# Arsham-001/tsu-emulator

Hardware: AMD Instinct MI355X
Metric: spin-updates/sec on L×L 2D Ising Gibbs sweep; achieved HBM GB/s vs peak (higher is better)
Workload: dtype int8

## Files before the change

### tsu-emulator_amd/csrc/ising2d_tiled.hip

```cpp
#include "ising2d.h"

#include <type_traits>
#include <vector>

typedef short v2s __attribute__((ext_vector_type(2)));
typedef unsigned short v2us __attribute__((ext_vector_type(2)));

struct TiledParams {
    const int8_t* src;
    int8_t* dst;
    long long pitch;
    int rows, nchunks;
    int cols;
    int q_shift;
    int tile_h;
    int flex_ty;
    int r_begin, r_end;
    long long row0, total_rows;
    int wrap_rows, ghost;
    int k;
    int tiles_x;
    int ty_first, ty_stride;
    uint32_t k0, k1, sweep0, tag_hi, tag_lo;
    uint32_t tblH0, tblH1, tblL0, tblL1;
// ... 205 lines not shown
template <int NO>
static __device__ __forceinline__ void edge_rows(const Rows2Ctx& c, int to_wrap, int tr, int& rga, int& rgb) {
    constexpr int SPAN = 2 * ((NO - 1 + 63) / NO) + 1;
    const int s_off = to_wrap > 0 ? c.rg_tile0 : c.rg_tile0 - c.total_rows;
    rga = tr + s_off;
    rgb = rga + 1;
    if (__builtin_expect((uint32_t)(to_wrap - 1) < (uint32_t)SPAN, 0)) {
        rga = tr + c.rg_tile0;
        asm volatile("" : "+v"(rga));
        rgb = rga + 1;
        if (rga >= c.total_rows) rga -= c.total_rows;
        if (rgb >= c.total_rows) rgb -= c.total_rows;
    }
}

constexpr int TBL2_OCTETS = 13;
constexpr uint32_t TBL2_LDS_ADDR = 0;

template <typename E, int NO>
struct TilePlanes {
    E* base;
    __device__ __forceinline__ E& at(int pl, int r, int o) const { return base[(2 * r + pl) * NO + o]; }
};

template <int NO, int KAPPA, int P0, bool EDGE, bool OPEN, bool SEAM>
static __device__ __forceinline__ void pair_step(const Rows2Ctx& c, const PhiloxKeys& K, uint32_t hs, uint32_t y0, uint32_t a, int rg, int to_wrap,
                                                 uint32_t cq) {
    constexpr int RS = 2 * NO * 8;
    constexpr int DO = (KAPPA ? NO : -NO) * 8;
    const uint64_t R0 = lds_ld<uint64_t>(a), R1 = lds_ld<uint64_t>(a + RS);
    const uint64_t R2 = lds_ld<uint64_t>(a + 2 * RS), R3 = lds_ld<uint64_t>(a + 3 * RS);
    const uint32_t A0 = SEAM ? 0u : (P0 ? lds_ld<volatile uint32_t>(a + RS + 8) : lds_ld<uint32_t>(a + RS - 4));
    const uint32_t A1 = SEAM ? 0u : (P0 ? lds_ld<uint32_t>(a + 2 * RS - 4) : lds_ld<volatile uint32_t>(a + 2 * RS + 8));
    const uint64_t Na = SEAM ? lds_ld<uint64_t>(a + RS + (P0 ? 8 : -8)) : 0ull;
    const uint64_t Nb = SEAM ? lds_ld<uint64_t>(a + 2 * RS + (P0 ? -8 : 8)) : 0ull;
    __builtin_amdgcn_sched_barrier(0);
    int rga = rg, rgb = rg + 1;
    if (EDGE) edge_rows<NO>(c, to_wrap, rg, rga, rgb);
    constexpr bool EARLY = !OPEN;
    auto counts = [&]() -> PairCounts {
        const uint32_t C0l = (uint32_t)R1, C0h = (uint32_t)(R1 >> 32), C1l = (uint32_t)R2, C1h = (uint32_t)(R2 >> 32);
        uint32_t S0l = P0 ? __builtin_amdgcn_alignbyte(C0h, C0l, 1) : __builtin_amdgcn_alignbyte(C0l, A0, 3);
        uint32_t S0h = P0 ? __builtin_amdgcn_alignbyte(A0, C0h, 1) : __builtin_amdgcn_alignbyte(C0h, C0l, 3);
        uint32_t S1l = P0 ? __builtin_amdgcn_alignbyte(C1l, A1, 3) : __builtin_amdgcn_alignbyte(C1h, C1l, 1);
        uint32_t S1h = P0 ? __builtin_amdgcn_alignbyte(C1h, C1l, 3) : __builtin_amdgcn_alignbyte(A1, C1h, 1);
        if (SEAM) {
            const uint64_t nxa = (Na & 0xFFull) << c.sh_next, pva = (Na >> c.sh_prev) & 0xFFull;
            const uint64_t nxb = (Nb & 0xFFull) << c.sh_next, pvb = (Nb >> c.sh_prev) & 0xFFull;
            const uint64_t Sa = P0 ? ((R1 >> 8) | nxa) : ((R1 << 8) | pva);
            const uint64_t Sb = P0 ? ((R2 << 8) | pvb) : ((R2 >> 8) | nxb);
            S0l = (uint32_t)Sa; S0h = (uint32_t)(Sa >> 32);
            S1l = (uint32_t)Sb; S1h = (uint32_t)(Sb >> 32);
        }
        const uint32_t ml = C0l + C1l, mh = C0h + C1h;
        return PairCounts{(uint32_t)R0 + ml + S0l, (uint32_t)(R0 >> 32) + mh + S0h, (uint32_t)R3 + ml + S1l, (uint32_t)(R3 >> 32) + mh + S1h};
    };
    PairCounts n;
    PairThr T;
    const u32x4 w0 = philox_vk(cq, (uint32_t)rga, c.rmask, y0, hs, c.tag_hi, K);
    if constexpr (EARLY) {
        __builtin_amdgcn_sched_barrier(0);
        n = counts();
        T = pair_thresholds(n, c.tbl2);
        __builtin_amdgcn_sched_barrier(0);
    }
    const u32x4 w1 = philox_vk(cq, (uint32_t)rgb, c.rmask, y0, hs, c.tag_hi, K);
    __builtin_amdgcn_sched_barrier(0);
    if constexpr (!EARLY) n = counts();
    const uint32_t cnt0l = n.c0l, cnt0h = n.c0h, cnt1l = n.c1l, cnt1h = n.c1h;
    u32x4 d0, d1;
    uint32_t edge_a = 0, edge_b = 0;
    if (OPEN) {
        const bool ea = rga == 0 || rga == c.last_row, eb = rgb == 0 || rgb == c.last_row;
        const bool la = !P0 && c.lft, ra = c.rgt && c.r_par == (uint32_t)P0, lb = P0 && c.lft, rb = c.rgt && c.r_par != (uint32_t)P0;
        d0 = compare_octet_open(w0, cnt0l, cnt0h, c, ea, la, ra);
        d1 = compare_octet_open(w1, cnt1l, cnt1h, c, eb, lb, rb);
        edge_a = (ea ? 1u : 0u) | (la ? 2u : 0u) | (ra ? 4u : 0u) | (c.r_slot << 4);
        edge_b = (eb ? 1u : 0u) | (lb ? 2u : 0u) | (rb ? 4u : 0u) | (c.r_slot << 4);
    } else {
        d0 = compare_octet_thr(w0, T.t);
        d1 = compare_octet_thr(w1, T.t + 4);
// ... 4 lines not shown
        if (has_zero_field(d1)) d1 = resolve_ties(d1, w1, cnt1l, cnt1h, c.s_thr, cq, (uint32_t)rgb & c.rmask, hs, c.tag_lo, c.k0, c.k1, edge_b);
    }
    uint64_t n0 = pack_flags(d0), n1 = pack_flags(d1);
    if (OPEN) {
        n0 = (rga < 0 || rga > c.last_row) ? 0 : (n0 & (P0 ? c.vm_o : c.vm_e));
        n1 = (rgb < 0 || rgb > c.last_row) ? 0 : (n1 & (P0 ? c.vm_e : c.vm_o));
    }
    if (SEAM) {
        n0 &= c.vm_e;
        n1 &= c.vm_e;
    }
    lds_st<uint64_t>(a + RS + DO, n0);
    lds_st<uint64_t>(a + 2 * RS + DO, n1);
}

template <int NO, int RL, int KAPPA, int P0, bool EDGE, bool OPEN, bool SEAM = false>
static __device__ __forceinline__ void sweep_pairs(const Rows2Ctx& c, const PhiloxKeys& K, uint32_t hs, uint32_t y0, uint32_t a, int rg, int n, bool tail,
                                                   uint32_t cq) {
    int to_wrap = EDGE ? c.wrap_tr - __builtin_amdgcn_readfirstlane(rg) : 0;
    bool live = true;
#pragma unroll 1
    for (int i = n; i >= 0; --i) {
        if (i == 0) live = tail;
        asm volatile("" : "+v"(a), "+v"(rg));
        if (live) pair_step<NO, KAPPA, P0, EDGE, OPEN, SEAM>(c, K, hs, y0, a, rg, to_wrap, cq);
        a += 2 * RL * 2 * NO * 8;
        rg += 2 * RL;
        to_wrap -= 2 * RL;
    }
}


static __device__ __forceinline__ uint32_t nib_shift_next(uint32_t X, uint32_t N) {
    const uint32_t hi = (N << 4) | __builtin_amdgcn_ubfe(X, 4u, 4u);
    return __builtin_amdgcn_alignbit(hi, X, 8);
}
static __device__ __forceinline__ uint32_t nib_shift_prev(uint32_t X, uint32_t M) {
    const uint32_t w = ((X << 4) & 0x10000000u) | (M >> 4);
    return __builtin_amdgcn_alignbit(X, w, 24);
}
static __device__ __forceinline__ uint32_t nib_shift_next_seam(uint32_t X, uint32_t N, int pos) {
    return nib_shift_next(X, 0u) | ((N & 0xFu) << pos);
}
// ... 76 lines not shown
static __device__ __forceinline__ void sweep_pairs_nib(const Rows2Ctx& c, const PhiloxKeys& K, uint32_t hs, uint32_t y0, uint32_t a, int rg, int n, bool tail,
                                                       uint32_t cq) {
    int to_wrap = EDGE ? c.wrap_tr - __builtin_amdgcn_readfirstlane(rg) : 0;
    bool live = true;
#pragma unroll 1
    for (int i = n; i >= 0; --i) {
        if (i == 0) live = tail;
        asm volatile("" : "+v"(a), "+v"(rg));
        if (live) pair_step_nib<NO, KAPPA, P0, EDGE, OPEN, SEAM>(c, K, hs, y0, a, rg, to_wrap, cq);
        a += 2 * RL * 2 * NO * 4;
        rg += 2 * RL;
        to_wrap -= 2 * RL;
    }
}

template <int NO, int RL, int KAPPA, int P0, bool EDGE, bool OPEN, bool SEAM, bool NIB>
static __device__ __forceinline__ void half_sweep(const Rows2Ctx& c, const PhiloxKeys& K, int TR, uint32_t sweep, int s, uint32_t a_thr, int al,
                                                  uint32_t cq) {
    constexpr int ES = NIB ? 4 : 8;
    const int hsi = 2 * s + KAPPA;
    __syncthreads();
    if (al < RL) {
        const int npairs = (TR - 2 - 2 * hsi) / 2;
        const int n = __builtin_amdgcn_readfirstlane(npairs / RL);
        const bool tail = al < npairs - n * RL;
        const uint32_t a = a_thr + (uint32_t)(hsi * 2 * NO * ES + (KAPPA ? 0 : NO * ES));
        int rg;
        if (EDGE) {
            rg = 1 + hsi + 2 * al;
        } else {
            int rgf = c.rg_tile0 + 1 + hsi;
            if (!OPEN && rgf >= c.total_rows) rgf -= c.total_rows;
            rg = rgf + 2 * al;
        }
        const uint32_t hs = 2u * sweep + (uint32_t)KAPPA;
        const uint32_t y0 = philox_y0(hs, c.k0);
        if constexpr (NIB) sweep_pairs_nib<NO, RL, KAPPA, P0, EDGE, OPEN, SEAM>(c, K, hs, y0, a, rg, n, tail, cq);
        else sweep_pairs<NO, RL, KAPPA, P0, EDGE, OPEN, SEAM>(c, K, hs, y0, a, rg, n, tail, cq);
    }
}

template <int NO, int RL, int P0, bool EDGE, bool OPEN, bool SEAM, bool NIB>
static __device__ __forceinline__ void sweep_generation(const Rows2Ctx& c, const PhiloxKeys& K, int TR, uint32_t sweep_g, int kg, uint32_t a_thr,
                                                        int al, uint32_t cq) {
#pragma unroll 1
    for (int s = 0; s < kg; ++s) {
        half_sweep<NO, RL, 0, P0, EDGE, OPEN, SEAM, NIB>(c, K, TR, sweep_g + (uint32_t)s, s, a_thr, al, cq);
        half_sweep<NO, RL, 1, P0, EDGE, OPEN, SEAM, NIB>(c, K, TR, sweep_g + (uint32_t)s, s, a_thr, al, cq);
    }
}

static __device__ __forceinline__ void xst(uint64_t* p, uint64_t v) { __hip_atomic_store(p, v, __ATOMIC_RELAXED, __HIP_MEMORY_SCOPE_AGENT); }
static __device__ __forceinline__ uint64_t xld(const uint64_t* p) { return __hip_atomic_load(p, __ATOMIC_RELAXED, __HIP_MEMORY_SCOPE_AGENT); }

struct ResidentParams {
    uint64_t* xbuf;
    uint32_t gen0;
    int* err;
    int n_gen, k_last, tiles_y;
    int wrap_y;
    int wrap_x;
    long long* dbg;
};

template <int HT, int WO, int THREADS, bool OPEN = false, bool RESIDENT = false, bool NIB = false>
static __device__ __forceinline__ void tile_body(const TiledParams& p, const int8_t* __restrict__ src, int8_t* __restrict__ dst,
                                                 const int k, const uint32_t sweep0, const int tx, const int ty, uint64_t* lds,
                                                 const PhiloxKeys& K, const ResidentParams* R = nullptr) {
    constexpr int NO = WO + 2;
    constexpr int RLMAX = THREADS / NO;
    int H, row_off;
    tile_rows(p, ty, row_off, H);
    const int TR = H + 4 * k;
    constexpr int RL = RLMAX;
    using E = typename std::conditional<NIB, uint32_t, uint64_t>::type;
    uint64_t* const guard = lds + TBL2_OCTETS;
    const TilePlanes<E, NO> P{reinterpret_cast<E*>(guard + 1)};
// ... 97 lines not shown
    const bool ragged = !OPEN && v_last != 0;
    const int seam_site = v_last - 1;
    const int seam_pos = NIB ? 8 * (seam_site & 3) + 4 * (seam_site >> 2) : 8 * seam_site, last_pos = NIB ? 28 : 56;
    c.sh_next = (ragged && cqi == p.nchunks - 1) ? seam_pos : last_pos;
    c.sh_prev = (ragged && cqi == 0) ? seam_pos : last_pos;
    int w0 = (q0 - 1) % p.nchunks;
    if (w0 < 0) w0 += p.nchunks;
    const bool seam = ragged && (w0 == 0 || w0 + NO - 1 >= p.nchunks - 1);
    if constexpr (OPEN) {
        asm volatile("v_mov_b32 %0, %1" : "=v"(c.tblH0) : "s"(p.tblH0));
        asm volatile("v_mov_b32 %0, %1" : "=v"(c.tblH1) : "s"(p.tblH1));
        asm volatile("v_mov_b32 %0, %1" : "=v"(c.tblL0) : "s"(p.tblL0));
        asm volatile("v_mov_b32 %0, %1" : "=v"(c.tblL1) : "s"(p.tblL1));
    }

    const int n_gen = RESIDENT ? R->n_gen : 1;
    long long tl0 = 0, tl[4] = {0, 0, 0, 0};
    const bool timing = RESIDENT && R->dbg && tid == 0;
    if (timing) tl0 = wall_clock64();
#define RES_MARK(q)                         \
    if (timing) {                           \
        const long long now_ = wall_clock64(); \
        tl[q] += now_ - tl0;                \
        tl0 = now_;                         \
    }
    volatile int& s_fail = *reinterpret_cast<volatile int*>(guard);
    if (RESIDENT && tid == 0) s_fail = 0;

    const int n_tb = 2 * k * WO, n_lr = H;
    const int xstride = 2 * n_tb + 2 * p.tile_h;
    const int wi = (p.nchunks + p.q_shift - q0) < WO ? (p.nchunks + p.q_shift - q0) : WO;
    constexpr uint64_t TAG_MASK = NIB ? 0xFFFFFFFF00000000ull : 0xFEFEull, FLAG_MASK = NIB ? 0x11111111ull : 0x0101010101010101ull;
// ... 52 lines not shown
            ad[it] = oc == 0 ? X_dl + e + w_l - 1 : (oc == wi + 1 ? X_dr + e : X_d + e + oc - 1);
            const bool col_ok = o == 0 ? has_l : (o == wi + 1 ? has_r : o <= wi);
            nu[it] = i < 2 * k * NO && has_u && col_ok;
            nd[it] = i < 2 * k * NO && has_d && col_ok;
            vu[it] = xld(au[it]);
            vd[it] = xld(ad[it]);
        }
#pragma unroll
        for (int it = 0; it < SI; ++it) {
            const int i = tid + it * THREADS, ic = i < n_lr ? i : 0;
            nl[it] = i < n_lr && has_l;
            nr[it] = i < n_lr && has_r;
            vl[it] = xld(X_l + 2 * n_tb + n_lr + ic);
            vr[it] = xld(X_r + 2 * n_tb + ic);
        }
        for (int spins = 0;; ++spins) {
            bool fresh = true;
#pragma unroll
            for (int it = 0; it < FI; ++it) {
                if (nu[it] && (vu[it] & TAG_MASK) != tag) { vu[it] = xld(au[it]); fresh = false; }
                if (nd[it] && (vd[it] & TAG_MASK) != tag) { vd[it] = xld(ad[it]); fresh = false; }
            }
#pragma unroll
            for (int it = 0; it < SI; ++it) {
                const int i = tid + it * THREADS, ic = i < n_lr ? i : 0;
                if (nl[it] && (vl[it] & TAG_MASK) != tag) { vl[it] = xld(X_l + 2 * n_tb + n_lr + ic); fresh = false; }
                if (nr[it] && (vr[it] & TAG_MASK) != tag) { vr[it] = xld(X_r + 2 * n_tb + ic); fresh = false; }
            }
            if (fresh) break;
            if (spins > (1 << 22) || ((spins & 0xFFF) == 0xFFF && __hip_atomic_load(R->err, __ATOMIC_RELAXED, __HIP_MEMORY_SCOPE_SYSTEM))) {
// ... 11 lines not shown
                if (nu[it]) P.at(1, r, o) = (E)(vu[it] & FLAG_MASK);
                if (nd[it]) P.at(1, 2 * k + H + r, o) = (E)(vd[it] & FLAG_MASK);
            }
        }
#pragma unroll
        for (int it = 0; it < SI; ++it) {
            const int i = tid + it * THREADS;
            if (i < n_lr) {
                if (nl[it]) P.at(1, 2 * k + i, 0) = (E)(vl[it] & FLAG_MASK);
                if (nr[it]) P.at(1, 2 * k + i, wi + 1) = (E)(vr[it] & FLAG_MASK);
            }
        }
        RES_MARK(3);
    };

    const int par0 = (int)((p.row0 + Rb + 1) & 1);
    const int form = 2 * (OPEN ? 0 : (seam ? 1 : (edge ? 2 : 3))) + par0;
    const uint32_t a_thr = lds_addr(P.base) + (uint32_t)((4 * al * NO + oct) * (int)sizeof(E));
    auto run_generation = [&](uint32_t sweep_g, int kg) {
#define TSU_FORM(P0, EDGE_, OPEN_, SEAM_) sweep_generation<NO, RL, P0, EDGE_, OPEN_, SEAM_, NIB>(c, K, TR, sweep_g, kg, a_thr, al, cq)
        if constexpr (OPEN) {
            if (par0) TSU_FORM(1, false, true, false);
            else TSU_FORM(0, false, true, false);
        } else {
            switch (form) {
                case 2: TSU_FORM(0, true, false, true); break;
                case 3: TSU_FORM(1, true, false, true); break;
                case 4: TSU_FORM(0, true, false, false); break;
                case 5: TSU_FORM(1, true, false, false); break;
                case 6: TSU_FORM(0, false, false, false); break;
                default: TSU_FORM(1, false, false, false); break;
            }
        }
#undef TSU_FORM
    };
    for (int gen = 0; gen < n_gen; ++gen) {
    const int kg = (RESIDENT && gen == n_gen - 1) ? R->k_last : k;
    const uint32_t sweep_g = sweep0 + (uint32_t)(gen * k);
    run_generation(sweep_g, kg);
    __syncthreads();
    if (RESIDENT && gen + 1 < n_gen) {
        publish(gen);
        fetch(gen);
        __syncthreads();
        if (s_fail) return;
    }
    RES_MARK(0);
    }
    if (timing)
        for (int q = 0; q < 4; ++q) R->dbg[4 * blockIdx.x + q] = tl[q];
#undef RES_MARK
    if (al < RLMAX && oct >= 1 && oct <= WO && q0 + oct - 1 < p.nchunks + p.q_shift) {
        int8_t* col = dst + 16 * (long long)cqi;
        int gpar = (int)((p.row0 + r0 + al) & 1);
#pragma unroll 2
        for (int hr = al; hr < H; hr += RLMAX) {
            const int rl = r0 + hr;
            if (rl < p.r_end) {
                uint64_t ev = P.at(gpar, 2 * k + hr, oct), od = P.at(gpar ^ 1, 2 * k + hr, oct);
                if (NIB) {
                    ev = (ev & 0x01010101ull) | (((ev >> 4) & 0x01010101ull) << 32);
                    od = (od & 0x01010101ull) | (((od >> 4) & 0x01010101ull) << 32);
                }
                const uint32_t e0 = perm(0u, 0x000001FFu, (uint32_t)ev), e1 = perm(0u, 0x000001FFu, (uint32_t)(ev >> 32));
                const uint32_t o0 = perm(0u, 0x000001FFu, (uint32_t)od), o1 = perm(0u, 0x000001FFu, (uint32_t)(od >> 32));
// ... 35 lines not shown
}

namespace {
constexpr int KMAX = 8;

struct TileVariant {
    int H, WO, threads;
    void (*kernel)(TiledParams);
    void (*resident)(ResidentLaunch);
    void (*open)(TiledParams);
    void (*resident_open)(ResidentLaunch);
    int nib;
    int per_cu;
};

size_t tile_lds_bytes(const TileVariant& tv, int TR) {
    const size_t es = tv.nib ? 4 : 8, NO = (size_t)tv.WO + 2;
    return 8 * TBL2_OCTETS + 8 + (((size_t)2 * TR * NO + NO + 1) * es + 7) / 8 * 8 + 8 + 25 * sizeof(uint64_t);
}
enum { V_64x512_T512 = 0, V_128x512_T512, V_128x512_T1024, V_256x512_T1024, V_128x256_T1024, V_64x512_T1024, V_64x256_T1024, V_32x256_T1024,
       V_N512x512_T1024, V_N256x512_T512 };
const TileVariant kVariants[] = {
    {64, 32, 512, k1_tiled2<64, 32, 512>, k1_resident<64, 32, 512>, k1_tiled2<64, 32, 512, 1, true>, nullptr, 0, 2},
    {128, 32, 512, k1_tiled2<128, 32, 512>, k1_resident<128, 32, 512>, k1_tiled2<128, 32, 512, 1, true>, nullptr, 0, 2},
    {128, 32, 1024, k1_tiled2<128, 32, 1024>, k1_resident<128, 32, 1024>, k1_tiled2<128, 32, 1024, 1, true>, k1_resident<128, 32, 1024, 1, true>, 0, 1},
    {256, 32, 1024, k1_tiled2<256, 32, 1024, 4>, k1_resident<256, 32, 1024, 4>, k1_tiled2<256, 32, 1024, 4, true>, k1_resident<256, 32, 1024, 4, true>, 0, 1},
    {128, 16, 1024, k1_tiled2<128, 16, 1024>, k1_resident<128, 16, 1024>, k1_tiled2<128, 16, 1024, 1, true>, k1_resident<128, 16, 1024, 1, true>, 0, 1},
    {64, 32, 1024, k1_tiled2<64, 32, 1024>, k1_resident<64, 32, 1024>, k1_tiled2<64, 32, 1024, 1, true>, k1_resident<64, 32, 1024, 1, true>, 0, 1},
    {64, 16, 1024, k1_tiled2<64, 16, 1024>, k1_resident<64, 16, 1024>, k1_tiled2<64, 16, 1024, 1, true>, k1_resident<64, 16, 1024, 1, true>, 0, 1},
    {32, 16, 1024, k1_tiled2<32, 16, 1024>, k1_resident<32, 16, 1024>, k1_tiled2<32, 16, 1024, 1, true>, k1_resident<32, 16, 1024, 1, true>, 0, 1},
    {512, 32, 1024, k1_tiled2<512, 32, 1024, 4, false, true>, k1_resident<512, 32, 1024, 4, false, true>, k1_tiled2<512, 32, 1024, 4, true, true>,
     k1_resident<512, 32, 1024, 4, true, true>, 1, 1},
    {256, 32, 512, k1_tiled2<256, 32, 512, 4, false, true>, nullptr, k1_tiled2<256, 32, 512, 4, true, true>, nullptr, 1, 2},
};
// ... 2 lines not shown
int ragged_shift(const tsu_ising2d* L, int WO) {
    if (!L->periodic || L->cols % 16 == 0) return 0;
    const int nch = (L->cols + 15) / 16, tiles_x = (nch + WO - 1) / WO;
    for (int shift = 1; shift < WO && shift < nch - 1; ++shift) {
        bool ok = true;
        for (int t = 0; t < tiles_x && ok; ++t) {
            const int s = t * WO + shift;
            if (s % nch == 0) ok = false;
            if (t < tiles_x - 1 && (s + WO) % nch == nch - 1) ok = false;
        }
        if (ok) return shift;
    }
    return -1;
}

size_t lds_share(const TileVariant& tv) { return (size_t)(160 / tv.per_cu) * 1024; }

int chip_cus(const tsu_ising2d* L) { return L->ctx->cus > 0 ? L->ctx->cus : 256; }

int lattice_env(const char* name, int dflt) {
    const char* e = getenv(name);
    return e ? atoi(e) : dflt;
}

double gen_time_us(const TileVariant& c, int h, double between) {
    const int pairs = (h + 4 * 8 - 2) / 2, waves = (pairs * (c.WO + 2) + 63) / 64;
    return 16.0 * (0.25 + (c.nib ? 1.06 : 1.0) * 0.225 * ((waves + 3) / 4)) + between;
}

template <typename P>
void pack_thresholds(P& p, const uint64_t table[25]) {
    for (int c = 0; c < 25; ++c) p.thr[c] = table[c];
    auto top16 = [](uint64_t thr) {
        uint32_t thi = (uint32_t)(thr >> 16);
        if (thi > 65535u) thi = 65535u;
        return thi ^ 0x8000u;
    };
    uint32_t t16[5], t3[8] = {0, 0, 0, 0, 0, 0, 0, 0};
// ... 38 lines not shown
            *v_out = cand[ci];
            *hmax_out = hmax;
        }
    }
    *t_out = best;
    return best_ty;
}

struct CallPlan {
    int v;
    int flex_ty, flex_h;
    int kmax;
    bool resident;
    int tile_h, tiles_y;
    int res_ext;
};

CallPlan plan_call(const tsu_ising2d* L, int n_sweeps, int part) {
    CallPlan c{};
    static const int env = lattice_env("TSU_TILE_VARIANT", -1);
    const bool forced = env >= 0 && env < kNumVariants;
    const int cus = chip_cus(L), nch = (L->cols + 15) / 16;
    const bool whole_lattice = L->ghost == 0 && L->total_rows == L->rows;
    int v;
    if (forced) {
        v = env;
    } else {
        const long long tx = (nch + 31) / 32;
        const long long n128 = ((L->rows + 127) / 128) * tx, n256 = ((L->rows + 255) / 256) * tx;
        if (n128 <= cus) v = V_128x512_T1024;
// ... 68 lines not shown
    if (whole && c.flex_ty > 0) {
        c.tile_h = c.flex_h;
        c.tiles_y = c.flex_ty;
    } else if (whole) {
        c.resident = nch % tv.WO == 0 && L->rows % tv.H == 0;
    } else {
        const int need = L->rows + 4 * (n_sweeps - c.kmax);
        int th = (need + c.tiles_y - 1) / c.tiles_y;
        th += th & 1;
        if (th < tv.H) th = tv.H;
        const int extra = th * c.tiles_y - L->rows;
        c.tile_h = th;
        c.res_ext = extra / 2;
        c.resident = nch % tv.WO == 0 && extra % 2 == 0 && c.res_ext <= L->ghost && tile_lds_bytes(tv, th + 4 * c.kmax) <= lds_share(tv);
    }
    return c;
}

int launch_tiles(const tsu_ising2d* L, const TileVariant& tv, int k, int left, int part, bool slab, TiledParams& p) {
    p.tile_h = tv.H;
    p.r_begin = 0;
    p.r_end = L->rows;
    if (part != TSU_PART_ALL) return (L->rows + tv.H - 1) / tv.H;
    if (!slab) {
        const long long slots = (long long)tv.per_cu * chip_cus(L);
        double best = 1e300;
        for (int th = 32; th <= 1024; th += 2) {
            if (th + 4 * KMAX > L->total_rows || tile_lds_bytes(tv, th + 4 * k) > lds_share(tv)) continue;
            const long long nt = (long long)((L->rows + th - 1) / th) * p.tiles_x, rounds = (nt + slots - 1) / slots;
            const double cost = (double)rounds * (th + 2 * k + 12);
// ... 3 lines not shown
            }
        }
        return (L->rows + p.tile_h - 1) / p.tile_h;
    }
    const int ext = 2 * (left - k);
    p.r_begin = -ext;
    p.r_end = L->rows + ext;
    const int base_ty = (L->rows + tv.H - 1) / tv.H;
    int th = (p.r_end - p.r_begin + base_ty - 1) / base_ty;
    th += th & 1;
    if (th >= tv.H && tile_lds_bytes(tv, th + 4 * k) <= lds_share(tv)) p.tile_h = th;
    return (p.r_end - p.r_begin + p.tile_h - 1) / p.tile_h;
}

void print_resident_timeline(const long long* d_dbg, int ntiles, int tiles_x, int tiles_y, int n_gen, int verbose) {
    std::vector<long long> h((size_t)4 * ntiles);
    (void)hipMemcpy(h.data(), d_dbg, h.size() * sizeof(long long), hipMemcpyDeviceToHost);
    static const char* const what[4] = {"sweeps", "publish", "wait", "fetch"};
    fprintf(stderr, "[tsu]   us per generation over %d tiles (mean / min / max):", ntiles);
    for (int q = 0; q < 4; ++q) {
        double sum = 0, lo = 1e30, hi = 0;
        for (int t = 0; t < ntiles; ++t) {
            const double v = h[(size_t)4 * t + q] / 100.0 / n_gen;
            sum += v;
            lo = v < lo ? v : lo;
            hi = v > hi ? v : hi;
        }
        fprintf(stderr, " %s %.1f / %.1f / %.1f%s", what[q], sum / ntiles, lo, hi, q < 3 ? "," : "\n");
    }
    if (verbose < 3) return;
    for (int x = 0; x < 8; ++x) {
        double sw = 0, wt = 0;
        int cnt = 0;
        for (int t = x; t < ntiles; t += 8, ++cnt) {
            sw += h[(size_t)4 * t] / 100.0 / n_gen;
            wt += h[(size_t)4 * t + 2] / 100.0 / n_gen;
        }
        if (cnt) fprintf(stderr, "[tsu]   xcd %d: sweeps %.2f wait %.2f\n", x, sw / cnt, wt / cnt);
    }
    if (verbose < 4) return;
    for (int y = 0; y < tiles_y; ++y) {
        fprintf(stderr, "[tsu]   row %3d:", y);
        for (int x = 0; x < tiles_x; ++x)
            fprintf(stderr, " %.1f/%.1f", h[(size_t)4 * (y * tiles_x + x)] / 100.0 / n_gen, h[(size_t)4 * (y * tiles_x + x) + 2] / 100.0 / n_gen);
        fprintf(stderr, "\n");
    }
}

int run_resident(tsu_ising2d* L, const CallPlan& c, TiledParams p, int n_sweeps, uint32_t sweep0, int fit_per_cu) {
    tsu_ctx* ctx = L->ctx;
    const TileVariant& tv = kVariants[c.v];
    void (*const res_kern)(ResidentLaunch) = L->periodic ? tv.resident : tv.resident_open;
    const int kmax = c.kmax, ntiles = p.tiles_x * c.tiles_y;
    const bool whole = L->wrap_rows || (!L->periodic && L->ghost == 0 && L->total_rows == L->rows);
    const size_t lds_bytes = tile_lds_bytes(tv, c.tile_h + 4 * kmax);
    const size_t xstride = (size_t)2 * (2 * kmax * tv.WO) + (size_t)2 * c.tile_h;
    const size_t xneed = (size_t)2 * ntiles * xstride;
    if (L->xbuf_cap < xneed * sizeof(uint64_t)) L->xsig = 0;
    TSU_HIP_TRY(ctx, ising2d_grow(L->d_xbuf, L->xbuf_cap, xneed * sizeof(uint64_t)));
    const uint64_t xsig = ((uint64_t)(c.v + 1) << 48) ^ ((uint64_t)ntiles << 28) ^ ((uint64_t)kmax << 20) ^ ((uint64_t)c.tile_h << 4) ^
                          ((uint64_t)c.flex_ty << 36) ^ (uint64_t)p.open;
    int* d_err = nullptr;
    if (const int rc = tsu_err_flag(ctx, L->h_err, &d_err); rc != TSU_OK) return rc;
    const int verbose = lattice_env("TSU_K1_VERBOSE", 0);
    const int chunk_max = whole ? 1024 * kmax : n_sweeps;
    for (int done = 0; done < n_sweeps;) {
        const int chunk = n_sweeps - done < chunk_max ? n_sweeps - done : chunk_max;
        ResidentLaunch P;
        p.k = kmax;
        p.sweep0 = sweep0 + (uint32_t)done;
// ... 9 lines not shown
        P.r.wrap_y = L->wrap_rows ? 1 : 0;
        P.r.wrap_x = L->periodic ? 1 : 0;
        P.r.xbuf = L->d_xbuf;
        const bool renumber = L->xsig != xsig || L->xgen + (uint32_t)((chunk + kmax - 1) / kmax) + 2u >= 16383u;
        if (renumber) {
            L->xrestarts += 1;
            L->xsig = xsig;
            L->xgen = 0;
        }
        P.r.gen0 = L->xgen + 1u;
        L->xgen += (uint32_t)((chunk + kmax - 1) / kmax);
        P.r.err = d_err;
        P.r.n_gen = (chunk + kmax - 1) / kmax;
        P.r.k_last = chunk - (P.r.n_gen - 1) * kmax;
        P.r.tiles_y = c.tiles_y;
        P.r.dbg = nullptr;
        long long* d_dbg = nullptr;
        if (verbose >= 2) {
            TSU_HIP_TRY(ctx, hipMalloc(&d_dbg, (size_t)4 * ntiles * sizeof(long long)));
            P.r.dbg = d_dbg;
        }
        if (verbose) {
            bool any_wrap = false;
            for (int ty = 0; ty < c.tiles_y && !any_wrap; ++ty) {
                long long rg0;
                any_wrap = tile_holds_wrap(P.t, ty, kmax, rg0);
            }
            fprintf(stderr, "[tsu] k1_resident variant %d: %d tiles (%d per CU fit), %d generations of %d sweeps, %zu KB of strips, row wrap: %s\n",
                    c.v, ntiles, fit_per_cu, P.r.n_gen, kmax, xneed * 8 / 1024, !any_wrap ? "none" : (wrap_by_mask(P.t) ? "mask" : "compare"));
        }
        {
            const int rcx = tsu_grid_exclusive_begin(ctx);
            if (rcx != TSU_OK) return rcx;
        }
        if (renumber) TSU_HIP_TRY(ctx, hipMemsetAsync(L->d_xbuf, 0, L->xbuf_cap, ctx->stream));
        TSU_HIP_TRY(ctx, tsu_launch_grid_sync(ctx, (const void*)res_kern, dim3((unsigned)ntiles), dim3((unsigned)tv.threads), &P, lds_bytes, ctx->stream,
                                              !whole));
        L->launches += 1;
        L->cur ^= 1;
        {
            const int rcx = tsu_grid_exclusive_end(ctx);
            if (rcx != TSU_OK) return rcx;
        }
        if (d_dbg) {
// ... 84 lines not shown
    p.ghost = L->ghost;
    p.tiles_x = (p.nchunks + tv.WO - 1) / tv.WO;
    p.q_shift = ragged_shift(L, tv.WO);
    p.r_begin = 0;
    p.r_end = L->rows;
    p.tile_h = tv.H;
    p.flex_ty = 0;
    ising2d_set_keys(p, seed, replica);
    pack_thresholds(p, L->table);
    p.open = L->periodic ? 0 : 1;
    TSU_HIP_TRY(ctx, tsu_func_allow_lds(ctx, (const void*)(L->periodic ? tv.kernel : tv.open), 160 * 1024));
    if (c.resident) {
        void (*const res_kern)(ResidentLaunch) = L->periodic ? tv.resident : tv.resident_open;
        TSU_HIP_TRY(ctx, tsu_func_allow_lds(ctx, (const void*)res_kern, 160 * 1024));
        int fit_per_cu = 0;
        TSU_HIP_TRY(ctx, tsu_func_blocks_per_cu(ctx, (const void*)res_kern, tv.threads, tile_lds_bytes(tv, (c.flex_ty > 0 ? c.tile_h : tv.H) + 4 * KMAX),
                                                &fit_per_cu));
        if ((long long)p.tiles_x * c.tiles_y <= (long long)fit_per_cu * ctx->cus) return run_resident(L, c, p, n_sweeps, sweep0, fit_per_cu);
    }
    return run_generations(L, c, p, n_sweeps, sweep0, part);
}

struct PlanesItem {
    int8_t* buf;
    long long pitch;
    int rows, cols, periodic;
    uint32_t k0, k1, tag_hi, tag_lo, sweep0;
    uint32_t tblH0, tblH1, tblL0, tblL1, t3H0, t3H1, t3L0, t3L1;
    uint64_t thr[25];
};

template <bool OPEN>
// ... 136 lines not shown
```

Measured before the change: 3258 billion.

## Precompute next generation's Philox blocks into LDS while waiting on halo exchange

In the resident periodic kernel, each lane now generates the Philox random words for the first few row-pairs of the next generation's first half-sweep during the inter-tile halo wait. It parks them in a new LDS region, and pair_step reads them back instead of recomputing. The goal is to hide RNG compute behind the grid-sync and halo-fetch latency. It costs extra LDS per block, which may reduce how many blocks fit per CU, and it adds a timeline slot for the fill phase.

```diff
diff --git a/tsu-emulator_amd/csrc/ising2d_tile_lds.h b/tsu-emulator_amd/csrc/ising2d_tile_lds.h
--- /dev/null
+++ b/tsu-emulator_amd/csrc/ising2d_tile_lds.h
@@ -0,0 +1,31 @@
+#pragma once
+#include <cstddef>
+
+constexpr int K1_TBL2_OCTETS = 13;
+constexpr int K1_PARK_MAX = 2;
+
+struct K1TileShape {
+    int WO, threads;
+    int nib;
+    int per_cu;
+};
+
+inline size_t k1_tile_lds_bytes(const K1TileShape& s, int TR) {
+    const size_t es = s.nib ? 4 : 8, NO = (size_t)s.WO + 2;
+    return 8 * K1_TBL2_OCTETS + 8 + (((size_t)2 * TR * NO + NO + 1) * es + 7) / 8 * 8 + 8 + 25 * 8;
+}
+inline size_t k1_lds_share(const K1TileShape& s) { return (size_t)(160 / s.per_cu) * 1024; }
+
+inline size_t k1_park_offset(const K1TileShape& s, int TR) { return (k1_tile_lds_bytes(s, TR) + 15) / 16 * 16; }
+inline size_t k1_park_bytes(const K1TileShape& s, int F) { return (size_t)F * s.threads * 32; }
+inline int k1_park_iterations(const K1TileShape& s, int TR_budget, int TR, bool periodic, int cap) {
+    if (s.nib || !periodic) return 0;
+    int F = cap < 0 ? 0 : (cap > K1_PARK_MAX ? K1_PARK_MAX : cap);
+    const int n = ((TR - 2) / 2) / (s.threads / (s.WO + 2));
+    if (F > n) F = n;
+    while (F > 0 && k1_park_offset(s, TR_budget) + k1_park_bytes(s, F) > k1_lds_share(s)) --F;
+    return F;
+}
+inline size_t k1_resident_lds_bytes(const K1TileShape& s, int TR, int F) {
+    return F > 0 ? k1_park_offset(s, TR) + k1_park_bytes(s, F) : k1_tile_lds_bytes(s, TR);
+}
diff --git a/tsu-emulator_amd/csrc/ising2d_tiled.hip b/tsu-emulator_amd/csrc/ising2d_tiled.hip
--- a/tsu-emulator_amd/csrc/ising2d_tiled.hip
+++ b/tsu-emulator_amd/csrc/ising2d_tiled.hip
@@ -1,10 +1,12 @@
 #include "ising2d.h"
+#include "ising2d_tile_lds.h"
 
 #include <type_traits>
 #include <vector>
 
 typedef short v2s __attribute__((ext_vector_type(2)));
 typedef unsigned short v2us __attribute__((ext_vector_type(2)));
+typedef uint32_t v4u __attribute__((ext_vector_type(4)));
 
 struct TiledParams {
     const int8_t* src;
@@ -243,7 +245,7 @@
     }
 }
 
-constexpr int TBL2_OCTETS = 13;
+constexpr int TBL2_OCTETS = K1_TBL2_OCTETS;
 constexpr uint32_t TBL2_LDS_ADDR = 0;
 
 template <typename E, int NO>
@@ -252,11 +254,17 @@
     __device__ __forceinline__ E& at(int pl, int r, int o) const { return base[(2 * r + pl) * NO + o]; }
 };
 
-template <int NO, int KAPPA, int P0, bool EDGE, bool OPEN, bool SEAM>
+template <int NO, int KAPPA, int P0, bool EDGE, bool OPEN, bool SEAM, int PARK = 0>
 static __device__ __forceinline__ void pair_step(const Rows2Ctx& c, const PhiloxKeys& K, uint32_t hs, uint32_t y0, uint32_t a, int rg, int to_wrap,
-                                                 uint32_t cq) {
+                                                 uint32_t cq, uint32_t slot = 0) {
     constexpr int RS = 2 * NO * 8;
     constexpr int DO = (KAPPA ? NO : -NO) * 8;
+    u32x4 w0, w1;
+    if constexpr (PARK != 0) {
+        const v4u p0 = lds_ld<v4u>(slot), p1 = lds_ld<v4u>(slot + PARK);
+        w0 = u32x4{p0.x, p0.y, p0.z, p0.w};
+        w1 = u32x4{p1.x, p1.y, p1.z, p1.w};
+    }
     const uint64_t R0 = lds_ld<uint64_t>(a), R1 = lds_ld<uint64_t>(a + RS);
     const uint64_t R2 = lds_ld<uint64_t>(a + 2 * RS), R3 = lds_ld<uint64_t>(a + 3 * RS);
     const uint32_t A0 = SEAM ? 0u : (P0 ? lds_ld<volatile uint32_t>(a + RS + 8) : lds_ld<uint32_t>(a + RS - 4));
@@ -286,14 +294,14 @@
     };
     PairCounts n;
     PairThr T;
-    const u32x4 w0 = philox_vk(cq, (uint32_t)rga, c.rmask, y0, hs, c.tag_hi, K);
+    if constexpr (PARK == 0) w0 = philox_vk(cq, (uint32_t)rga, c.rmask, y0, hs, c.tag_hi, K);
     if constexpr (EARLY) {
         __builtin_amdgcn_sched_barrier(0);
         n = counts();
         T = pair_thresholds(n, c.tbl2);
         __builtin_amdgcn_sched_barrier(0);
     }
-    const u32x4 w1 = philox_vk(cq, (uint32_t)rgb, c.rmask, y0, hs, c.tag_hi, K);
+    if constexpr (PARK == 0) w1 = philox_vk(cq, (uint32_t)rgb, c.rmask, y0, hs, c.tag_hi, K);
     __builtin_amdgcn_sched_barrier(0);
     if constexpr (!EARLY) n = counts();
     const uint32_t cnt0l = n.c0l, cnt0h = n.c0h, cnt1l = n.c1l, cnt1h = n.c1h;
@@ -328,6 +336,8 @@
     lds_st<uint64_t>(a + 2 * RS + DO, n1);
 }
 
+template <int RL>
+constexpr int lane_row_step() { return 2 * RL; }
 template <int NO, int RL, int KAPPA, int P0, bool EDGE, bool OPEN, bool SEAM = false>
 static __device__ __forceinline__ void sweep_pairs(const Rows2Ctx& c, const PhiloxKeys& K, uint32_t hs, uint32_t y0, uint32_t a, int rg, int n, bool tail,
                                                    uint32_t cq) {
@@ -338,9 +348,9 @@
         if (i == 0) live = tail;
         asm volatile("" : "+v"(a), "+v"(rg));
         if (live) pair_step<NO, KAPPA, P0, EDGE, OPEN, SEAM>(c, K, hs, y0, a, rg, to_wrap, cq);
-        a += 2 * RL * 2 * NO * 8;
-        rg += 2 * RL;
-        to_wrap -= 2 * RL;
+        a += lane_row_step<RL>() * 2 * NO * 8;
+        rg += lane_row_step<RL>();
+        to_wrap -= lane_row_step<RL>();
     }
 }
 
@@ -447,38 +457,71 @@
     }
 }
 
-template <int NO, int RL, int KAPPA, int P0, bool EDGE, bool OPEN, bool SEAM, bool NIB>
-static __device__ __forceinline__ void half_sweep(const Rows2Ctx& c, const PhiloxKeys& K, int TR, uint32_t sweep, int s, uint32_t a_thr, int al,
-                                                  uint32_t cq) {
+struct HalfSweepStart {
+    int n;
+    bool tail;
+    uint32_t a;
+    int rg;
+    uint32_t hs, y0;
+};
+template <int NO, int RL, int KAPPA, bool EDGE, bool OPEN, bool NIB>
+static __device__ __forceinline__ HalfSweepStart half_sweep_start(const Rows2Ctx& c, int TR, uint32_t sweep, int s, uint32_t a_thr, int al) {
     constexpr int ES = NIB ? 4 : 8;
     const int hsi = 2 * s + KAPPA;
+    HalfSweepStart st;
+    const int npairs = (TR - 2 - 2 * hsi) / 2;
+    st.n = __builtin_amdgcn_readfirstlane(npairs / RL);
+    st.tail = al < npairs - st.n * RL;
+    st.a = a_thr + (uint32_t)(hsi * 2 * NO * ES + (KAPPA ? 0 : NO * ES));
+    if (EDGE) {
+        st.rg = 1 + hsi + 2 * al;
+    } else {
+        int rgf = c.rg_tile0 + 1 + hsi;
+        if (!OPEN && rgf >= c.total_rows) rgf -= c.total_rows;
+        st.rg = rgf + 2 * al;
+    }
+    st.hs = 2u * sweep + (uint32_t)KAPPA;
+    st.y0 = philox_y0(st.hs, c.k0);
+    return st;
+}
+
+template <int NO, int RL, int KAPPA, int P0, bool EDGE, bool OPEN, bool SEAM, bool NIB, int PARK = 0>
+static __device__ __forceinline__ void half_sweep(const Rows2Ctx& c, const PhiloxKeys& K, int TR, uint32_t sweep, int s, uint32_t a_thr, int al,
+                                                  uint32_t cq, int npark = 0, uint32_t slot = 0) {
     __syncthreads();
     if (al < RL) {
-        const int npairs = (TR - 2 - 2 * hsi) / 2;
-        const int n = __builtin_amdgcn_readfirstlane(npairs / RL);
-        const bool tail = al < npairs - n * RL;
-        const uint32_t a = a_thr + (uint32_t)(hsi * 2 * NO * ES + (KAPPA ? 0 : NO * ES));
-        int rg;
-        if (EDGE) {
-            rg = 1 + hsi + 2 * al;
+        const HalfSweepStart st = half_sweep_start<NO, RL, KAPPA, EDGE, OPEN, NIB>(c, TR, sweep, s, a_thr, al);
+        if constexpr (NIB) {
+            sweep_pairs_nib<NO, RL, KAPPA, P0, EDGE, OPEN, SEAM>(c, K, st.hs, st.y0, st.a, st.rg, st.n, st.tail, cq);
         } else {
-            int rgf = c.rg_tile0 + 1 + hsi;
-            if (!OPEN && rgf >= c.total_rows) rgf -= c.total_rows;
-            rg = rgf + 2 * al;
-        }
-        const uint32_t hs = 2u * sweep + (uint32_t)KAPPA;
-        const uint32_t y0 = philox_y0(hs, c.k0);
-        if constexpr (NIB) sweep_pairs_nib<NO, RL, KAPPA, P0, EDGE, OPEN, SEAM>(c, K, hs, y0, a, rg, n, tail, cq);
-        else sweep_pairs<NO, RL, KAPPA, P0, EDGE, OPEN, SEAM>(c, K, hs, y0, a, rg, n, tail, cq);
-    }
-}
-
-template <int NO, int RL, int P0, bool EDGE, bool OPEN, bool SEAM, bool NIB>
+            uint32_t a = st.a;
+            int rg = st.rg, n = st.n;
+            if constexpr (PARK != 0 && KAPPA == 0) {
+                static_assert(!EDGE && !OPEN && !SEAM, "parked Philox blocks: the plain loop only");
+                if (s == 0 && npark > 0) {
+                    const int np = npark < n ? npark : n;
+#pragma unroll 1
+                    for (int j = 0; j < np; ++j) {
+                        asm volatile("" : "+v"(a), "+v"(rg), "+v"(slot));
+                        pair_step<NO, KAPPA, P0, EDGE, OPEN, SEAM, PARK>(c, K, st.hs, st.y0, a, rg, 0, cq, slot);
+                        a += lane_row_step<RL>() * 2 * NO * 8;
+                        rg += lane_row_step<RL>();
+                        slot += 2 * PARK;
+                    }
+                    n -= np;
+                }
+            }
+            sweep_pairs<NO, RL, KAPPA, P0, EDGE, OPEN, SEAM>(c, K, st.hs, st.y0, a, rg, n, st.tail, cq);
+        }
+    }
+}
+
+template <int NO, int RL, int P0, bool EDGE, bool OPEN, bool SEAM, bool NIB, int PARK = 0>
 static __device__ __forceinline__ void sweep_generation(const Rows2Ctx& c, const PhiloxKeys& K, int TR, uint32_t sweep_g, int kg, uint32_t a_thr,
-                                                        int al, uint32_t cq) {
+                                                        int al, uint32_t cq, int npark = 0, uint32_t slot = 0) {
 #pragma unroll 1
     for (int s = 0; s < kg; ++s) {
-        half_sweep<NO, RL, 0, P0, EDGE, OPEN, SEAM, NIB>(c, K, TR, sweep_g + (uint32_t)s, s, a_thr, al, cq);
+        half_sweep<NO, RL, 0, P0, EDGE, OPEN, SEAM, NIB, PARK>(c, K, TR, sweep_g + (uint32_t)s, s, a_thr, al, cq, npark, slot);
         half_sweep<NO, RL, 1, P0, EDGE, OPEN, SEAM, NIB>(c, K, TR, sweep_g + (uint32_t)s, s, a_thr, al, cq);
     }
 }
@@ -494,6 +537,8 @@
     int wrap_y;
     int wrap_x;
     long long* dbg;
+    int park;
+    uint32_t park_off;
 };
 
 template <int HT, int WO, int THREADS, bool OPEN = false, bool RESIDENT = false, bool NIB = false>
@@ -621,8 +666,16 @@
         asm volatile("v_mov_b32 %0, %1" : "=v"(c.tblL1) : "s"(p.tblL1));
     }
 
+    const int par0 = (int)((p.row0 + Rb + 1) & 1);
+    const int form = 2 * (OPEN ? 0 : (seam ? 1 : (edge ? 2 : 3))) + par0;
+    const uint32_t a_thr = lds_addr(P.base) + (uint32_t)((4 * al * NO + oct) * (int)sizeof(E));
+    constexpr int PARK = (RESIDENT && !NIB && !OPEN) ? THREADS * 16 : 0;
+    const int npark_tile = (PARK != 0 && form >= 6) ? R->park : 0;
+    const uint32_t park_slot = PARK != 0 ? R->park_off + 16u * (uint32_t)tid : 0u;
+    auto generation_sweep = [&](int gen) { return sweep0 + (uint32_t)(gen * k); };
+
     const int n_gen = RESIDENT ? R->n_gen : 1;
-    long long tl0 = 0, tl[4] = {0, 0, 0, 0};
+    long long tl0 = 0, tl[5] = {0, 0, 0, 0, 0};
     const bool timing = RESIDENT && R->dbg && tid == 0;
     if (timing) tl0 = wall_clock64();
 #define RES_MARK(q)                         \
@@ -705,6 +758,26 @@
             vl[it] = xld(X_l + 2 * n_tb + n_lr + ic);
             vr[it] = xld(X_r + 2 * n_tb + ic);
         }
+        if constexpr (PARK != 0) {
+            __builtin_amdgcn_sched_barrier(0);
+            if (npark_tile > 0 && al < RL) {
+                const HalfSweepStart st = half_sweep_start<NO, RL, 0, false, false, false>(c, TR, generation_sweep(gen + 1), 0, a_thr, al);
+                const int np = npark_tile < st.n ? npark_tile : st.n;
+                int rg = st.rg;
+                uint32_t slot = park_slot;
+#pragma unroll 1
+                for (int j = 0; j < np; ++j) {
+                    const u32x4 w0 = philox_vk(cq, (uint32_t)rg, c.rmask, st.y0, st.hs, c.tag_hi, K);
+                    const u32x4 w1 = philox_vk(cq, (uint32_t)rg + 1u, c.rmask, st.y0, st.hs, c.tag_hi, K);
+                    lds_st<v4u>(slot, v4u{w0.x, w0.y, w0.z, w0.w});
+                    lds_st<v4u>(slot + PARK, v4u{w1.x, w1.y, w1.z, w1.w});
+                    rg += lane_row_step<RL>();
+                    slot += 2 * PARK;
+                }
+            }
+            RES_MARK(4);
+            __builtin_amdgcn_sched_barrier(0);
+        }
         for (int spins = 0;; ++spins) {
             bool fresh = true;
 #pragma unroll
@@ -746,30 +819,27 @@
         RES_MARK(3);
     };
 
-    const int par0 = (int)((p.row0 + Rb + 1) & 1);
-    const int form = 2 * (OPEN ? 0 : (seam ? 1 : (edge ? 2 : 3))) + par0;
-    const uint32_t a_thr = lds_addr(P.base) + (uint32_t)((4 * al * NO + oct) * (int)sizeof(E));
-    auto run_generation = [&](uint32_t sweep_g, int kg) {
-#define TSU_FORM(P0, EDGE_, OPEN_, SEAM_) sweep_generation<NO, RL, P0, EDGE_, OPEN_, SEAM_, NIB>(c, K, TR, sweep_g, kg, a_thr, al, cq)
+    auto run_generation = [&](uint32_t sweep_g, int kg, int npark) {
+#define TSU_FORM(P0, EDGE_, OPEN_, SEAM_, PARK_) \
+    sweep_generation<NO, RL, P0, EDGE_, OPEN_, SEAM_, NIB, PARK_>(c, K, TR, sweep_g, kg, a_thr, al, cq, npark, park_slot)
         if constexpr (OPEN) {
-            if (par0) TSU_FORM(1, false, true, false);
-            else TSU_FORM(0, false, true, false);
+            if (par0) TSU_FORM(1, false, true, false, 0);
+            else TSU_FORM(0, false, true, false, 0);
         } else {
             switch (form) {
-                case 2: TSU_FORM(0, true, false, true); break;
-                case 3: TSU_FORM(1, true, false, true); break;
-                case 4: TSU_FORM(0, true, false, false); break;
-                case 5: TSU_FORM(1, true, false, false); break;
-                case 6: TSU_FORM(0, false, false, false); break;
-                default: TSU_FORM(1, false, false, false); break;
+                case 2: TSU_FORM(0, true, false, true, 0); break;
+                case 3: TSU_FORM(1, true, false, true, 0); break;
+                case 4: TSU_FORM(0, true, false, false, 0); break;
+                case 5: TSU_FORM(1, true, false, false, 0); break;
+                case 6: TSU_FORM(0, false, false, false, PARK); break;
+                default: TSU_FORM(1, false, false, false, PARK); break;
             }
         }
 #undef TSU_FORM
     };
     for (int gen = 0; gen < n_gen; ++gen) {
     const int kg = (RESIDENT && gen == n_gen - 1) ? R->k_last : k;
-    const uint32_t sweep_g = sweep0 + (uint32_t)(gen * k);
-    run_generation(sweep_g, kg);
+    run_generation(generation_sweep(gen), kg, gen > 0 ? npark_tile : 0);
     __syncthreads();
     if (RESIDENT && gen + 1 < n_gen) {
         publish(gen);
@@ -780,7 +850,7 @@
     RES_MARK(0);
     }
     if (timing)
-        for (int q = 0; q < 4; ++q) R->dbg[4 * blockIdx.x + q] = tl[q];
+        for (int q = 0; q < 5; ++q) R->dbg[5 * blockIdx.x + q] = tl[q];
 #undef RES_MARK
     if (al < RLMAX && oct >= 1 && oct <= WO && q0 + oct - 1 < p.nchunks + p.q_shift) {
         int8_t* col = dst + 16 * (long long)cqi;
@@ -846,10 +916,8 @@
     int per_cu;
 };
 
-size_t tile_lds_bytes(const TileVariant& tv, int TR) {
-    const size_t es = tv.nib ? 4 : 8, NO = (size_t)tv.WO + 2;
-    return 8 * TBL2_OCTETS + 8 + (((size_t)2 * TR * NO + NO + 1) * es + 7) / 8 * 8 + 8 + 25 * sizeof(uint64_t);
-}
+K1TileShape lds_shape(const TileVariant& tv) { return K1TileShape{tv.WO, tv.threads, tv.nib, tv.per_cu}; }
+size_t tile_lds_bytes(const TileVariant& tv, int TR) { return k1_tile_lds_bytes(lds_shape(tv), TR); }
 enum { V_64x512_T512 = 0, V_128x512_T512, V_128x512_T1024, V_256x512_T1024, V_128x256_T1024, V_64x512_T1024, V_64x256_T1024, V_32x256_T1024,
        V_N512x512_T1024, V_N256x512_T512 };
 const TileVariant kVariants[] = {
@@ -882,7 +950,7 @@
     return -1;
 }
 
-size_t lds_share(const TileVariant& tv) { return (size_t)(160 / tv.per_cu) * 1024; }
+size_t lds_share(const TileVariant& tv) { return k1_lds_share(lds_shape(tv)); }
 
 int chip_cus(const tsu_ising2d* L) { return L->ctx->cus > 0 ? L->ctx->cus : 256; }
 
@@ -890,6 +958,12 @@
     const char* e = getenv(name);
     return e ? atoi(e) : dflt;
 }
+
+int resident_park(const TileVariant& tv, int tile_h, int k, bool periodic) {
+    static const int cap = lattice_env("TSU_K1_PARK", K1_PARK_MAX);
+    return k1_park_iterations(lds_shape(tv), tile_h + 4 * KMAX, tile_h + 4 * k, periodic, cap);
+}
+size_t resident_lds_bytes(const TileVariant& tv, int TR, int park) { return k1_resident_lds_bytes(lds_shape(tv), TR, park); }
 
 double gen_time_us(const TileVariant& c, int h, double between) {
     const int pairs = (h + 4 * 8 - 2) / 2, waves = (pairs * (c.WO + 2) + 63) / 64;
@@ -958,6 +1032,7 @@
     bool resident;
     int tile_h, tiles_y;
     int res_ext;
+    int park;
 };
 
 CallPlan plan_call(const tsu_ising2d* L, int n_sweeps, int part) {
@@ -1056,6 +1131,7 @@
         c.res_ext = extra / 2;
         c.resident = nch % tv.WO == 0 && extra % 2 == 0 && c.res_ext <= L->ghost && tile_lds_bytes(tv, th + 4 * c.kmax) <= lds_share(tv);
     }
+    if (c.resident) c.park = resident_park(tv, c.tile_h, c.kmax, L->periodic);
     return c;
 }
 
@@ -1089,35 +1165,39 @@
 }
 
 void print_resident_timeline(const long long* d_dbg, int ntiles, int tiles_x, int tiles_y, int n_gen, int verbose) {
-    std::vector<long long> h((size_t)4 * ntiles);
+    constexpr int NQ = 5;
+    std::vector<long long> h((size_t)NQ * ntiles);
     (void)hipMemcpy(h.data(), d_dbg, h.size() * sizeof(long long), hipMemcpyDeviceToHost);
-    static const char* const what[4] = {"sweeps", "publish", "wait", "fetch"};
+    static const char* const what[NQ] = {"sweeps", "publish", "wait", "fetch", "fill"};
     fprintf(stderr, "[tsu]   us per generation over %d tiles (mean / min / max):", ntiles);
-    for (int q = 0; q < 4; ++q) {
+    for (int q = 0; q < NQ; ++q) {
         double sum = 0, lo = 1e30, hi = 0;
         for (int t = 0; t < ntiles; ++t) {
-            const double v = h[(size_t)4 * t + q] / 100.0 / n_gen;
+            const double v = h[(size_t)NQ * t + q] / 100.0 / n_gen;
             sum += v;
             lo = v < lo ? v : lo;
             hi = v > hi ? v : hi;
         }
-        fprintf(stderr, " %s %.1f / %.1f / %.1f%s", what[q], sum / ntiles, lo, hi, q < 3 ? "," : "\n");
+        fprintf(stderr, " %s %.1f / %.1f / %.1f%s", what[q], sum / ntiles, lo, hi, q < NQ - 1 ? "," : "\n");
     }
     if (verbose < 3) return;
     for (int x = 0; x < 8; ++x) {
-        double sw = 0, wt = 0;
+        double sw = 0, wt = 0, fl = 0;
         int cnt = 0;
         for (int t = x; t < ntiles; t += 8, ++cnt) {
-            sw += h[(size_t)4 * t] / 100.0 / n_gen;
-            wt += h[(size_t)4 * t + 2] / 100.0 / n_gen;
-        }
-        if (cnt) fprintf(stderr, "[tsu]   xcd %d: sweeps %.2f wait %.2f\n", x, sw / cnt, wt / cnt);
+            sw += h[(size_t)NQ * t] / 100.0 / n_gen;
+            wt += h[(size_t)NQ * t + 2] / 100.0 / n_gen;
+            fl += h[(size_t)NQ * t + 4] / 100.0 / n_gen;
+        }
+        if (cnt) fprintf(stderr, "[tsu]   xcd %d: sweeps %.2f wait %.2f fill %.2f\n", x, sw / cnt, wt / cnt, fl / cnt);
     }
     if (verbose < 4) return;
     for (int y = 0; y < tiles_y; ++y) {
         fprintf(stderr, "[tsu]   row %3d:", y);
-        for (int x = 0; x < tiles_x; ++x)
-            fprintf(stderr, " %.1f/%.1f", h[(size_t)4 * (y * tiles_x + x)] / 100.0 / n_gen, h[(size_t)4 * (y * tiles_x + x) + 2] / 100.0 / n_gen);
+        for (int x = 0; x < tiles_x; ++x) {
+            const long long* t = &h[(size_t)NQ * (y * tiles_x + x)];
+            fprintf(stderr, " %.1f/%.1f/%.1f", t[0] / 100.0 / n_gen, t[2] / 100.0 / n_gen, t[4] / 100.0 / n_gen);
+        }
         fprintf(stderr, "\n");
     }
 }
@@ -1128,7 +1208,7 @@
     void (*const res_kern)(ResidentLaunch) = L->periodic ? tv.resident : tv.resident_open;
     const int kmax = c.kmax, ntiles = p.tiles_x * c.tiles_y;
     const bool whole = L->wrap_rows || (!L->periodic && L->ghost == 0 && L->total_rows == L->rows);
-    const size_t lds_bytes = tile_lds_bytes(tv, c.tile_h + 4 * kmax);
+    const size_t lds_bytes = resident_lds_bytes(tv, c.tile_h + 4 * kmax, c.park);
     const size_t xstride = (size_t)2 * (2 * kmax * tv.WO) + (size_t)2 * c.tile_h;
     const size_t xneed = (size_t)2 * ntiles * xstride;
     if (L->xbuf_cap < xneed * sizeof(uint64_t)) L->xsig = 0;
@@ -1168,10 +1248,12 @@
         P.r.n_gen = (chunk + kmax - 1) / kmax;
         P.r.k_last = chunk - (P.r.n_gen - 1) * kmax;
         P.r.tiles_y = c.tiles_y;
+        P.r.park = c.park;
+        P.r.park_off = (uint32_t)k1_park_offset(lds_shape(tv), c.tile_h + 4 * kmax);
         P.r.dbg = nullptr;
         long long* d_dbg = nullptr;
         if (verbose >= 2) {
-            TSU_HIP_TRY(ctx, hipMalloc(&d_dbg, (size_t)4 * ntiles * sizeof(long long)));
+            TSU_HIP_TRY(ctx, hipMalloc(&d_dbg, (size_t)5 * ntiles * sizeof(long long)));
             P.r.dbg = d_dbg;
         }
         if (verbose) {
@@ -1180,8 +1262,8 @@
                 long long rg0;
                 any_wrap = tile_holds_wrap(P.t, ty, kmax, rg0);
             }
-            fprintf(stderr, "[tsu] k1_resident variant %d: %d tiles (%d per CU fit), %d generations of %d sweeps, %zu KB of strips, row wrap: %s\n",
-                    c.v, ntiles, fit_per_cu, P.r.n_gen, kmax, xneed * 8 / 1024, !any_wrap ? "none" : (wrap_by_mask(P.t) ? "mask" : "compare"));
+            fprintf(stderr, "[tsu] k1_resident variant %d: %d tiles (%d per CU fit), %d generations of %d sweeps, %zu KB of strips, parked: %d, row wrap: %s\n",
+                    c.v, ntiles, fit_per_cu, P.r.n_gen, kmax, xneed * 8 / 1024, c.park, !any_wrap ? "none" : (wrap_by_mask(P.t) ? "mask" : "compare"));
         }
         {
             const int rcx = tsu_grid_exclusive_begin(ctx);
@@ -1296,8 +1378,8 @@
         void (*const res_kern)(ResidentLaunch) = L->periodic ? tv.resident : tv.resident_open;
         TSU_HIP_TRY(ctx, tsu_func_allow_lds(ctx, (const void*)res_kern, 160 * 1024));
         int fit_per_cu = 0;
-        TSU_HIP_TRY(ctx, tsu_func_blocks_per_cu(ctx, (const void*)res_kern, tv.threads, tile_lds_bytes(tv, (c.flex_ty > 0 ? c.tile_h : tv.H) + 4 * KMAX),
-                                                &fit_per_cu));
+        TSU_HIP_TRY(ctx, tsu_func_blocks_per_cu(ctx, (const void*)res_kern, tv.threads,
+                                                resident_lds_bytes(tv, (c.flex_ty > 0 ? c.tile_h : tv.H) + 4 * KMAX, c.park), &fit_per_cu));
         if ((long long)p.tiles_x * c.tiles_y <= (long long)fit_per_cu * ctx->cus) return run_resident(L, c, p, n_sweeps, sweep0, fit_per_cu);
     }
     return run_generations(L, c, p, n_sweeps, sweep0, part);
```

Result: no change. 3277 billion (median of 6 runs) (+0.6%).
